# ebarnett2/batotp

Measured on AMD Instinct MI355X. Metric: constraint-evaluated waypoints/sec + traversal-time err vs CPU ref, higher is better.
Workload: dtype f64

## Files before the change

batotp_amd/capi.py:

```python
from __future__ import annotations

import ctypes as C
import os
from typing import Optional, Sequence

import numpy as np

_HERE = os.path.dirname(os.path.abspath(__file__))
_ROOT = os.path.dirname(_HERE)
HIP_LIB_PATH = os.path.join(_HERE, "csrc", "libbatotp_hip.so")

MAX_JOINTS = 8
MAX_CART = 8

ROBOT_KUKA, ROBOT_UR, ROBOT_RR, ROBOT_CSPR3DOF, ROBOT_GENJNT = 1, 2, 3, 4, 5
F_JNT_ACC_ON, F_TRQ_ON, F_CART_VEL_ON, F_CART_ACC_ON = 1 << 0, 1 << 1, 1 << 2, 1 << 3
F_PARALLEL, F_PAR2SER, F_HOST_TRIG, F_NO_SAMPLES, F_COMPACT_SPLINES = 1 << 4, 1 << 5, 1 << 6, 1 << 7, 1 << 8
F_CURVES_IN_PLACE = 1 << 9
F_MVC_IN_CURVES = 1 << 10
F_SVD = 1 << 11
ST_MAX_INTEG_TIME, ST_CAPACITY, ST_BISECT_FAIL = 1 << 0, 1 << 1, 1 << 2
ST_NONFINITE, ST_SHORT, ST_SEG_ERROR = 1 << 3, 1 << 4, 1 << 5

PATH_JOINT, PATH_CART, PATH_BOTH = 1, 2, 3
# ... 767 lines not shown
        self.L.check(self.lib.batotp_hip_output_ms(self.handle, C.byref(v)), "output_ms")
        return float(v.value)


def output_from_rows(ctx: "Context", rows_list, sres, n_theta: int, n_cart: int, n_trq: int) -> Output:
    return Output.from_rows(ctx, rows_list, sres, n_theta, n_cart, n_trq)


def fwdkin_chain(ctx: "Context", chain: KinChain, theta_list: Sequence[np.ndarray], host_trig: bool = True):
    ctx.library.need_kin()
    arrs = [np.ascontiguousarray(t, dtype=np.float64) for t in theta_list]
    for a in arrs:
        assert a.ndim == 2 and a.shape[0] == chain.n_links, (a.shape, chain.n_links)
    n_pts = np.ascontiguousarray([a.shape[1] for a in arrs], dtype=np.int64)
    flat = np.ascontiguousarray(np.concatenate([a.ravel() for a in arrs])) if arrs else np.zeros(0)
    out = np.empty(3 * int(n_pts.sum()), dtype=np.float64)
    ctx.library.check(ctx.library.lib.batotp_hip_fwdkin_chain(ctx.handle, C.byref(chain), F_HOST_TRIG if host_trig else 0, len(arrs),
                                                              n_pts.ctypes.data_as(C.POINTER(C.c_int64)), _dptr(flat), _dptr(out)), "fwdkin_chain")
    res, at = [], 0
    for n in n_pts:
        res.append(out[at: at + 3 * int(n)].reshape(3, int(n)))
        at += 3 * int(n)
    return res


def sdiv_kat(ctx: "Context", a: np.ndarray, b: np.ndarray):
    a = np.ascontiguousarray(a, dtype=np.float64); b = np.ascontiguousarray(b, dtype=np.float64)
    q = np.empty_like(a); w = np.empty(a.size, dtype=np.int32)
    ctx.library.check(ctx.library.lib.batotp_hip_sdiv_kat(ctx.handle, a.size, _dptr(a), _dptr(b), _dptr(q),
                                                          w.ctypes.data_as(C.POINTER(C.c_int32))), "sdiv_kat")
    return q, w.astype(bool)


def out_segmax_kat(ctx: "Context", segs):
    n1 = np.ascontiguousarray([len(x) for x in segs], dtype=np.int32)
    flat = np.ascontiguousarray(np.concatenate([np.asarray(x, dtype=np.int32) for x in segs]), dtype=np.int32)
    ctx.library.check(ctx.library.lib.batotp_hip_out_segmax_kat(ctx.handle, len(segs), n1.ctypes.data_as(C.POINTER(C.c_int32)),
                                                                flat.ctypes.data_as(C.POINTER(C.c_int32))), "out_segmax_kat")
    return np.split(flat, np.cumsum(n1)[:-1])


def spline_lanes_kat(ctx: "Context", y: np.ndarray):
    y = np.ascontiguousarray(y, dtype=np.float64)
    sol, seq = np.empty_like(y), np.empty_like(y)
    redone = C.c_int32(0)
    ctx.library.check(ctx.library.lib.batotp_hip_spline_lanes_kat(ctx.handle, y.size, _dptr(y), _dptr(sol), _dptr(seq), C.byref(redone)),
                      "spline_lanes_kat")
    return sol, seq, int(redone.value)


def div6_kat(ctx: "Context", a: np.ndarray) -> np.ndarray:
    a = np.ascontiguousarray(a, dtype=np.float64)
    q = np.empty_like(a)
    ctx.library.check(ctx.library.lib.batotp_hip_div6_kat(ctx.handle, a.size, _dptr(a), _dptr(q)), "div6_kat")
    return q


class Batch:

    def __init__(self, ctx: Context, prob: Problem, n_knots: Sequence[int], max_steps: int):
        self.ctx, self.lib, self.L = ctx, ctx.library.lib, ctx.library
        self.prob = prob
        self.n_knots = np.ascontiguousarray(n_knots, dtype=np.int64)
        self.n_paths = int(self.n_knots.size)
        self.max_steps = int(max_steps)
        self.handle = C.c_void_p()
# ... 152 lines not shown
```

batotp_amd/csrc/batotp_hip.hip:

```cpp
#include <hip/hip_runtime.h>

#include <algorithm>
#include <cmath>
#include <cstdio>
#include <cstdlib>
#include <cstring>
#include <new>
#include <thread>
#include <type_traits>
#include <vector>

#include "batotp_hip.h"
#include "batotp_models.h"
#include "kernels.hip.h"
#include "sweep1.hip.h"
#include "sweep8.hip.h"
#include "sweep8_fwd.hip.h"
#include "pointwise_va.hip.h"
#include "spline_stream.hip.h"
#include "spline_tile.hip.h"
#include "spline_lanes.hip.h"
#include "resample.hip.h"
#include "output.hip.h"
#include "audit.hip.h"
#include "kin_chain.hip.h"
#include "invdyn.hip.h"
#include "stretch.hip.h"
#include "tscale.hip.h"
#include "stretch_rounds.h"

static inline unsigned seriesBlock(int64_t series)
{
   const int64_t lanes = (series + 255) / 256;
   return (unsigned)(lanes < 4 ? 4 : (lanes > 64 ? 64 : lanes));
}

static inline bool seriesLanesPay(int64_t series) { return series <= 4096; }

using namespace bk;

constexpr int BATOTP_CERT_HOLD_DEFAULT = 3;

static thread_local char g_err[512] = "";

static int hipFail(hipError_t e, const char *what)
// ... 500 lines not shown
   HIP_TRY(hipMemsetAsync(dB, 0xff, sz, st));
   HIP_TRY(hipMemsetAsync(dFlag, 0, sizeof(int), st));
   hipLaunchKernelGGL(k_spline_series_lanes, dim3(1), dim3(64), 0, st, 1, dOff, dOff, dCnt, dy, 1, dA, dFlag);
   HIP_TRY(hipGetLastError());
   hipLaunchKernelGGL(k_spline_series, dim3(1), dim3(seriesBlock(1)), 0, st, 1, dOff, dOff, dCnt, dy, 1, dA, dFlag);
   HIP_TRY(hipGetLastError());
   hipLaunchKernelGGL(k_spline_series, dim3(1), dim3(seriesBlock(1)), 0, st, 1, dOff, dOff, dCnt, dy, 1, dB, (const int *)nullptr);
   HIP_TRY(hipGetLastError());
   HIP_TRY(hipMemcpyAsync(sol, dA, sz, hipMemcpyDeviceToHost, st));
   HIP_TRY(hipMemcpyAsync(sol_seq, dB, sz, hipMemcpyDeviceToHost, st));
   int flag = 0;
   HIP_TRY(hipMemcpyAsync(&flag, dFlag, sizeof(int), hipMemcpyDeviceToHost, st));
   HIP_TRY(hipStreamSynchronize(st));
   *redone = flag;
   return BATOTP_OK;
}

extern "C" int batotp_hip_sdiv_kat(batotp_ctx *ctx, int64_t n, const double *a, const double *b, double *q, int32_t *in_window)
{
   if (!ctx || n <= 0 || !a || !b || !q || !in_window) return BATOTP_ERR_ARG;
   int rc = bind(ctx);
   if (rc) return rc;
   double *d = nullptr;
   const size_t sz = sizeof(double) * (size_t)n;
   HIP_TRY(hipMalloc((void **)&d, 4 * sz));
   hipMemcpyAsync(d, a, sz, hipMemcpyHostToDevice, ctx->stream);
   hipMemcpyAsync(d + n, b, sz, hipMemcpyHostToDevice, ctx->stream);
   hipLaunchKernelGGL(k_kat_sdiv, dim3((unsigned)((n + 255) / 256)), dim3(256), 0, ctx->stream, n, d, d + n, d + 2 * n, reinterpret_cast<int *>(d + 3 * n));
   hipMemcpyAsync(q, d + 2 * n, sz, hipMemcpyDeviceToHost, ctx->stream);
   hipMemcpyAsync(in_window, d + 3 * n, sizeof(int32_t) * (size_t)n, hipMemcpyDeviceToHost, ctx->stream);
   hipError_t e = hipStreamSynchronize(ctx->stream);
   hipFree(d);
   if (e != hipSuccess) return hipFail(e, "sdiv_kat");
   return BATOTP_OK;
}

static int xferReserve(batotp_ctx *ctx, size_t bytes, double **out)
{
   if (ctx->xfer.cap < bytes)
   {
      if (ctx->xfer.p) { hipFree(ctx->xfer.p); ctx->xfer.p = nullptr; ctx->xfer.cap = 0; }
      const size_t want = std::max(bytes, (size_t)1 << 20);
      hipError_t e = hipMalloc(&ctx->xfer.p, want);
      if (e != hipSuccess) { hipFail(e, "hipMalloc(staging)"); (void)hipGetLastError(); return BATOTP_ERR_ALLOC; }
      ctx->xfer.cap = want;
   }
   *out = static_cast<double *>(ctx->xfer.p);
   return BATOTP_OK;
}

static int dynDim(const batotp_problem *prob)
{
   if (!(prob->flags & BATOTP_F_TRQ_ON)) return 0;
   return (prob->flags & BATOTP_F_PARALLEL) ? prob->n_cart : prob->n_joints;
}

extern "C" int batotp_hip_batch_destroy(batotp_batch *b)
{
   if (!b) return BATOTP_OK;
   if (b->ctx) hipSetDevice(b->ctx->device);
   if (b->ctx && b->k3Pending) hipStreamSynchronize(b->ctx->stream2);
   if (b->dFwd == b->dRev) b->dFwd = nullptr;
   void *ptrs[] = {b->dP, b->dPinfo, b->dY, b->dSC, b->dCoef, b->dSamp, b->dDyn, b->dTrig, b->dMvc, b->dRev, b->dFwd, b->dRes, b->dStage, b->dSink, b->dElim, b->dKM, b->dUp, b->dModel, b->dJTrig, b->dTileOff, b->dDirty, b->dEdge, b->dProf, b->dOrder};
   for (void *p : ptrs)
      if (p) hipFree(p);
   for (int k = 0; k < 5; ++k)
// ... 1102 lines not shown
```

batotp_amd/csrc/device_math.h:

```cpp
#pragma once
#include <hip/hip_runtime.h>

namespace bk
{

__device__ __forceinline__ double dmin(double a, double b) { return (b < a) ? b : a; }
__device__ __forceinline__ double dmax(double a, double b) { return (a < b) ? b : a; }
__device__ __forceinline__ int sgn(double v) { return (0.0 < v) - (v < 0.0); }

constexpr double kInf = __builtin_huge_val();

constexpr int DPP_QUAD_XOR1 = 0xB1;
constexpr int DPP_QUAD_XOR2 = 0x4E;
constexpr int DPP_ROW_HALF_MIRROR = 0x141;
constexpr int DPP_ROW_MIRROR = 0x140;
constexpr int DPP_ROW_ROR8 = 0x128;

template <int CTRL>
__device__ __forceinline__ double dpp_mov(double v)
{
   const int lo = __builtin_amdgcn_mov_dpp(__double2loint(v), CTRL, 0xf, 0xf, true);
   const int hi = __builtin_amdgcn_mov_dpp(__double2hiint(v), CTRL, 0xf, 0xf, true);
   return __hiloint2double(hi, lo);
}
template <int CTRL>
__device__ __forceinline__ int dpp_mov(int v)
{
   return __builtin_amdgcn_mov_dpp(v, CTRL, 0xf, 0xf, true);
}

__device__ __forceinline__ double vmin_f64(double a, double b)
{
   double r;
   asm("v_min_f64 %0, %1, %2" : "=v"(r) : "v"(a), "v"(b));
   return r;
}
__device__ __forceinline__ double vmax_f64(double a, double b)
{
   double r;
   asm("v_max_f64 %0, %1, %2" : "=v"(r) : "v"(a), "v"(b));
   return r;
}

template <int G>
__device__ __forceinline__ double grp_min(double v)
{
   if (G == 1) return v;
   v = vmin_f64(v, dpp_mov<DPP_QUAD_XOR1>(v));
   if (G >= 4) v = vmin_f64(v, dpp_mov<DPP_QUAD_XOR2>(v));
   if (G >= 8) v = vmin_f64(v, dpp_mov<DPP_ROW_HALF_MIRROR>(v));
   if (G == 16) v = vmin_f64(v, dpp_mov<DPP_ROW_MIRROR>(v));
   return v;
}
template <int G>
__device__ __forceinline__ double grp_max(double v)
{
   if (G == 1) return v;
   v = vmax_f64(v, dpp_mov<DPP_QUAD_XOR1>(v));
   if (G >= 4) v = vmax_f64(v, dpp_mov<DPP_QUAD_XOR2>(v));
   if (G >= 8) v = vmax_f64(v, dpp_mov<DPP_ROW_HALF_MIRROR>(v));
   if (G == 16) v = vmax_f64(v, dpp_mov<DPP_ROW_MIRROR>(v));
   return v;
}
__device__ __forceinline__ double vmin_f64_raw(double a, double b)
{
   double r;
   asm("v_min_f64 %0, %1, %2" : "=v"(r) : "v"(a), "v"(b));
   return r;
}
__device__ __forceinline__ double vmax_f64_raw(double a, double b)
{
   double r;
   asm("v_max_f64 %0, %1, %2" : "=v"(r) : "v"(a), "v"(b));
   return r;
// ... 64 lines not shown
```

batotp_amd/csrc/sweep8.hip.h:

```cpp
#pragma once
#include "kernels.hip.h"
#include "mvc_window.h"
#include "knot_window.h"

#ifdef S8_PROFILE
#define S8_CNT(k, v) pc[k] += (double)(v)
#define S8_TICK(var) const unsigned long long var = __builtin_readcyclecounter()
#define S8_CYC(k, a, b) pc[k] += (double)((b) - (a))
#else
#define S8_CNT(k, v)
#define S8_TICK(var)
#define S8_CYC(k, a, b)
#endif

namespace bk
{

constexpr int S8_BLOCK = 256;
#define S8_ANY(x) (__builtin_amdgcn_ballot_w64(x) != 0)
#define S8_RARE(x) __builtin_expect(S8_ANY(x), 0)

__device__ __forceinline__ bool s8_ratio_lt_fast(double num, double den, double thr, bool &decided)
{
   const double p = thr * den;
   const bool ok = (p > 1e-290) & (p < 1e290);
   const bool lt = num < p * (1.0 - 1e-14), gt = num > p * (1.0 + 1e-14);
   decided = ok & (lt | gt);
   return lt;
}
__device__ __forceinline__ void s8_ratio_lt_pair(double num1, double num2, double den, bool &lt1, bool &dec1, bool &lt2, bool &dec2)
{
   constexpr double T1 = .001, T2 = 1e-20;
   const bool ok = (den > 1e-260) & (den < 1e260);
   lt1 = num1 < den * (T1 * (1.0 - 1e-14));
   lt2 = num2 < den * (T2 * (1.0 - 1e-14));
   dec1 = ok & (lt1 | (num1 > den * (T1 * (1.0 + 1e-14))));
   dec2 = ok & (lt2 | (num2 > den * (T2 * (1.0 + 1e-14))));
}


__global__ void k_kat_sdiv(int64_t n, const double *__restrict__ a, const double *__restrict__ b, double *__restrict__ q, int *__restrict__ inWindow)
{
   const int64_t i = (int64_t)blockIdx.x * blockDim.x + threadIdx.x;
   if (i >= n) return;
   const bool ok = sdiv_window(a[i]) & sdiv_window(b[i]);
   inWindow[i] = ok ? 1 : 0;
   q[i] = ok ? sdiv_by(a[i], b[i], sdiv_rcp(b[i])) : a[i] / b[i];
}

constexpr int DPP_QUAD_XOR3 = 0x1B;
__device__ __forceinline__ double s8_rcp2(double d)
{
   double r = __builtin_amdgcn_rcp(d);
   r = __builtin_fma(__builtin_fma(-d, r, 1.0), r, r);
   return __builtin_fma(__builtin_fma(-d, r, 1.0), r, r);
}
__device__ __forceinline__ double s8_absmax(double x, double floorv)
{
   double r;
   asm("v_max_f64 %0, |%1|, %2" : "=v"(r) : "v"(x), "v"(floorv));
   return r;
}
__device__ __forceinline__ void s8_certify(bool jOn, double thD, double thD2, double rD, bool rOk, double amaxq, double thrV, double thrA,
                                           double sddotMax, double &lowFact, double &sdotH, double &sdotL, double &sdotTry,
                                           double &sdotGood, int &nGood, int &nIter)
{
   constexpr double BIG = 1e300, TINY = 1e-300;
   const double xTop = sdotH * sdotH;
   const bool use = jOn && !(fabs(thD) < thrV);
   const double aur = amaxq * fabs(rD), mr = thD2 * rD;
   const double er = aur + fabs(mr) * xTop;
   const bool lineOk = rOk & (aur < 1e100) & (fabs(mr) < 1e100) & (er < 1e100);
   const bool have = use & lineOk;
   const double au = have ? aur : BIG;
   const double mj = have ? mr : 0.0;
   const double ej = use ? (lineOk ? er : kInf) : 0.0;
   const double uMin = grp_min<8>(au);
   const double eMax = grp_max<8>(ej);
   const double sMin2 = dmin(uMin, sddotMax);
   const bool standing = jOn && !use && !(fabs(thD2) < thrA);
   double xForce = kInf;
   if (S8_RARE(standing)) xForce = grp_min<8>(standing ? amaxq / fabs(thD2) : kInf);
   double xs = (au + sddotMax) * s8_rcp2(s8_absmax(mj, TINY));
#define S8_PAIR(AUI, MI) xs = vmin_f64(xs, (au + (AUI)) * s8_rcp2(s8_absmax(mj - (MI), TINY)))
   {
      const double a1 = dpp_mov<DPP_QUAD_XOR1>(au), m1 = dpp_mov<DPP_QUAD_XOR1>(mj);
      S8_PAIR(a1, m1);
      const double a2 = dpp_mov<DPP_QUAD_XOR2>(au), m2 = dpp_mov<DPP_QUAD_XOR2>(mj);
      S8_PAIR(a2, m2);
      const double a3 = dpp_mov<DPP_QUAD_XOR3>(au), m3 = dpp_mov<DPP_QUAD_XOR3>(mj);
      S8_PAIR(a3, m3);
      const double a7 = dpp_mov<DPP_ROW_HALF_MIRROR>(au), m7 = dpp_mov<DPP_ROW_HALF_MIRROR>(mj);
      S8_PAIR(a7, m7);
      const double a6 = dpp_mov<DPP_QUAD_XOR1>(a7), m6 = dpp_mov<DPP_QUAD_XOR1>(m7);
      S8_PAIR(a6, m6);
      const double a5 = dpp_mov<DPP_QUAD_XOR2>(a7), m5 = dpp_mov<DPP_QUAD_XOR2>(m7);
      S8_PAIR(a5, m5);
      const double a4 = dpp_mov<DPP_QUAD_XOR3>(a7), m4 = dpp_mov<DPP_QUAD_XOR3>(m7);
      S8_PAIR(a4, m4);
   }
#undef S8_PAIR
   xs = grp_min<8>(xs);
   const double xstar = dmin(xs, 4.0 * xTop);
   const double R = eMax * s8_rcp2(sMin2 > 0.0 ? sMin2 : 1.0);
   const double band = (R * 0x1p-40) * xstar;
   const bool forceFirst = xForce < xstar - band;
   const double xThr = forceFirst ? xForce : xstar;
   const double bandThr = forceFirst ? -1.0 : band;
   const bool sane = (sddotMax == sddotMax) & (eMax == eMax) & (xstar == xstar) & (R == R) & (R < 0x1p30) & (sMin2 > 1e-100) & (eMax < 1e100) &
                     (xTop > 1e-100) & (xTop < 1e100) & (xstar > 1e-100) & (forceFirst | (xForce > xstar + band));
   if (sane)
   {
      int it = nIter;
      bool inBand = false, more = true;
      for (;;)
      {
         const double c = sdotTry, d = c * c - xThr;
         inBand = !((fabs(d) > bandThr) & (c > 1e-100));
         more = more & !inBand & (d > 0.0) & (it < 90);
         if (!S8_ANY(more)) break;
         const double lf2 = lowFact * 2.0;
         const double lo = dmax(.999 * 0.0, (1.0 - lf2) * c);
         lowFact = more ? lf2 : lowFact;
         sdotH = more ? c : sdotH;
         sdotL = more ? lo : sdotL;
         sdotTry = .5 * (sdotH + sdotL);
         it += more ? 1 : 0;
      }
      const bool bisect = !inBand & (it < 90);
      sdotGood = bisect ? sdotTry : sdotGood;
      nGood = bisect ? 1 : nGood;
      sdotL = bisect ? sdotTry : sdotL;
      it += bisect ? 1 : 0;
      sdotTry = .5 * (sdotH + sdotL);
      const double convThr = 1e-3 * (1.0 + 3e-14);
      more = bisect;
      for (;;)
      {
         const double c = sdotTry, d = c * c - xThr;
         const bool viol = d > 0.0;
         const bool goesOn = viol | (fabs(c - sdotL) > convThr * c);
         more = more & (fabs(d) > bandThr) & goesOn & (it < 90);
         if (!S8_ANY(more)) break;
         sdotH = (more & viol) ? c : sdotH;
         sdotL = (more & !viol) ? c : sdotL;
         sdotTry = .5 * (sdotH + sdotL);
         it += more ? 1 : 0;
      }
      sdotGood = bisect ? sdotL : sdotGood;
      nIter = it;
   }
}

template <int G, int FEAT, int DIR>
__global__ void __launch_bounds__(S8_BLOCK, G == 8 ? 2 : 1) k_sweep8(SweepArgs a)
{
   static_assert(FEAT == -1 || FEAT == 0, "velocity / acceleration-only problems");
   static_assert(G == 8 || G == 4, "lanes per path");
   constexpr int PER = 8 / G;
   __shared__ double lim[6][8];
   __shared__ double rk[7][6];
   __shared__ double2 pts[S8_BLOCK / G][4];
   __shared__ double2 vw[S8_BLOCK / G][8];
   if (threadIdx.x < 42)
   {
      const double tab[42] = {0, 0, 0, 0, 0, 0,
                              BK_B00, 0, 0, 0, 0, 0,
                              BK_B01, BK_B11, 0, 0, 0, 0,
                              BK_B02, BK_B12, BK_B22, 0, 0, 0,
                              BK_B03, BK_B13, BK_B23, BK_B33, 0, 0,
                              BK_B04, BK_B14, BK_B24, BK_B34, BK_B44, 0,
                              BK_B05, BK_B15, BK_B25, BK_B35, BK_B45, BK_B55};
      (&rk[0][0])[threadIdx.x] = tab[threadIdx.x];
   }
   stage_limits(a.dP, lim);

// ... 103 lines not shown
   unsigned status = t.status;
   int nfail = t.nfail;
   double sdotCur = t.sdotCur;
   double sddotL = t.sddotL, sddotH = t.sddotH;

   double v1 = 0, v2 = 0, v3 = 0, v4 = 0, v5 = 0;
   double w1 = 0, w2 = 0, w3 = 0, w4 = 0, w5 = 0, w6 = 0;
   double sPrev = s0v, sdPrev = v0, sCurPt = s0v, sdCurPt = v0;
   double sCur = s0v;

   const int iMax = (maxIntegSteps > 0x3ffffff0) ? 0x3ffffff0 : (int)maxIntegSteps;
   const int capI = (int)cap;
   const int revStartI = (revStart > 0x3fffffff) ? 0x3fffffff : (int)revStart;
#define S8_CURVE_FULL(i) ((i) >= capI || (DIR == 1 && (i) + 64 >= revStartI + segM))

   {
      const int idx0 = (DIR == 1) ? 0 : capI - 1;
      if (writer) { out[idx0] = make_double2(s0v, v0); mypts[idx0 & 3] = make_double2(s0v, v0); }
   }
   int flushedTo = (DIR == 1) ? 0 : capI;

   const double floorV = 0.0 / absh;
   int nPts = 0, i = 1;
   unsigned endStatus = 0;
   int st = (DIR == 1) ? -1 : 0;
   constexpr int PH_FIRST = 0, PH_ENDED = 1, PH_CHECK = 2, PH_DEAD = 3, PH_CERT = 4;
   constexpr bool CERT = DIR == -1 && PER == 1;
   const int holdC = a.holdc;
   int phase = PH_ENDED;
   if (S8_CURVE_FULL(i)) { endStatus = BATOTP_ST_CAPACITY; phase = PH_DEAD; }
   double sN = 0, wN = 0;
   double lowFact = .01, sdotGood = 0, sdotL = 0, sdotH = 0, sdotTry = 0;
   int nGood = 0, nIter = 0;
   bool wild = !(fabs(v0) < kInf) | !(fabs(w0) < kInf);
   bool stageFailed = false;
   const int hold = a.hold;
#ifdef S8_PROFILE
   double pc[16];
   for (int k = 0; k < 16; ++k) pc[k] = 0;
   const unsigned long long tLoop0 = __builtin_readcyclecounter();
#endif

   for (;;)
   {
      const unsigned long long mAlive = __ballot(phase != PH_DEAD);
      if (mAlive == 0) break;
      const unsigned long long mWait = __ballot(phase < PH_CHECK);
      const bool startNow = (mWait == mAlive) || (__popcll(mWait) * 8 >= __popcll(mAlive) * hold);
      S8_CNT(0, 1); S8_CNT(13, __popcll(mAlive) / G);
      if (CERT)
      {
         const unsigned long long mCert = __ballot(phase == PH_CERT);
         if (mCert != 0)
         {
            const bool progress = (startNow && mWait != 0) || ((mAlive & ~mWait & ~mCert) != 0);
            if (__popcll(mCert) * 8 >= __popcll(mAlive) * holdC || !progress)
            {
               S8_TICK(tF0);
               S8_CNT(11, 1); S8_CNT(15, __popcll(mCert) / G);
               if (phase == PH_CERT)
               {
                  s8_certify(jOn[0], thD[0], thD2[0], rD[0], rOk[0], amax[0], thrV, thrA, sddotMax, lowFact, sdotH, sdotL, sdotTry, sdotGood,
                             nGood, nIter);
                  phase = PH_CHECK;
               }
               S8_TICK(tF1);
               S8_CYC(14, tF0, tF1);
            }
         }
      }
      S8_TICK(tA);
      if (startNow && mWait != 0)
      {
         S8_CNT(1, 1); S8_CNT(2, __popcll(mWait) / G);
         if (phase < PH_CHECK)
         {
            {
               phase = PH_FIRST;
               const double vN = sdotCur;
               wild |= !(fabs(vN) < kInf) | !(fabs(wN) < kInf);
               {
                  double *slotV = reinterpret_cast<double *>(myvw + ((unsigned)st < 6u ? st : 7));
                  double *slotW = reinterpret_cast<double *>(myvw + (((unsigned)st < 6u && !stageFailed) ? st : 7)) + 1;
                  *slotV = vN;
                  *slotW = wN;
               }
               const bool stepEnd = (st == 6);
               st = stepEnd ? st : st + 1;
               if (S8_ANY(stepEnd))
               {
                  S8_CNT(8, 1);
                  if (stepEnd)
                  {
                     const double wE = stageFailed ? w6 : wN;
                     s0v = sN; v0 = vN; w0 = wE; w6 = wE;
                     sPrev = sCurPt; sdPrev = sdCurPt;
                     sCurPt = s0v; sdCurPt = v0;
                     const int idx = (DIR == 1) ? i : capI - 1 - i;
                     mypts[idx & 3] = make_double2(s0v, v0);
                     st = (DIR == 1) ? 0 : 1;
                     const bool fin = sCur * DIR > sLast;
                     const bool late = !fin && (i > iMax);
                     nPts = fin ? i + 1 : nPts;
                     i = (fin || late) ? i : i + 1;
                     const bool full = !fin && !late && S8_CURVE_FULL(i);
                     endStatus = late ? (unsigned)BATOTP_ST_MAX_INTEG_TIME : (full ? (unsigned)BATOTP_ST_CAPACITY : endStatus);
                     phase = (fin || late || full) ? PH_DEAD : phase;
                     const bool chunk = !fin && ((DIR == 1) ? ((idx & 3) == 3) : ((idx & 3) == 0));
                     if (S8_ANY(chunk))
                     {
                        if (chunk)
                        {
                           const int base = idx & ~3;
// ... 20 lines not shown
                        st = 1;
                     }
                  }
               }
               const double *bc = rk[st];
               double sdotT = 0, sddotT = 0;
               {
                  const double2 q1 = myvw[1], q2 = myvw[2], q3 = myvw[3], q4 = myvw[4], q5 = myvw[5];
                  v1 = q1.x; w1 = q1.y; v2 = q2.x; w2 = q2.y; v3 = q3.x; w3 = q3.y; v4 = q4.x; w4 = q4.y; v5 = q5.x; w5 = q5.y;
               }
               bool slowDiv = false;
#pragma unroll
               for (int q = 0; q < PER; ++q) slowDiv |= jOn[q] && fabs(thD[q]) > thrV && !(rOk[q] & sdiv_window(vmax[q]));
               const bool odd = S8_RARE(wild | slowDiv);
               if (!odd)
               {
                  sdotT += bc[0] * v0; sddotT += bc[0] * w0;
                  sdotT += bc[1] * v1; sddotT += bc[1] * w1;
                  sdotT += bc[2] * v2; sddotT += bc[2] * w2;
                  sdotT += bc[3] * v3; sddotT += bc[3] * w3;
                  sdotT += bc[4] * v4; sddotT += bc[4] * w4;
                  sdotT += bc[5] * v5; sddotT += bc[5] * w5;
               }
               else
               {
                  sdotT += bc[0] * v0; sddotT += bc[0] * w0;
                  { const double a1 = sdotT + bc[1] * v1, b1 = sddotT + bc[1] * w1; sdotT = (st > 1) ? a1 : sdotT; sddotT = (st > 1) ? b1 : sddotT; }
                  { const double a2 = sdotT + bc[2] * v2, b2 = sddotT + bc[2] * w2; sdotT = (st > 2) ? a2 : sdotT; sddotT = (st > 2) ? b2 : sddotT; }
                  { const double a3 = sdotT + bc[3] * v3, b3 = sddotT + bc[3] * w3; sdotT = (st > 3) ? a3 : sdotT; sddotT = (st > 3) ? b3 : sddotT; }
                  { const double a4 = sdotT + bc[4] * v4, b4 = sddotT + bc[4] * w4; sdotT = (st > 4) ? a4 : sdotT; sddotT = (st > 4) ? b4 : sddotT; }
                  { const double a5 = sdotT + bc[5] * v5, b5 = sddotT + bc[5] * w5; sdotT = (st > 5) ? a5 : sdotT; sddotT = (st > 5) ? b5 : sddotT; }
               }
               sN = s0v + h * sdotT;
               double vN = v0 + h * sddotT;
               vN = dmax(vN, floorV);
               sCur = sN;

               if (DIR == 1)
               {
#include "sweep8_mvcwalk.inc"
                  const double tauM = (sCur - mS0) / (mS1 - mS0);
                  const double sdotMVC = dmax(mD0 + tauM * (mD1 - mD0), sdotMin);
                  vN = (vN > sdotMVC) ? sdotMVC : vN;
               }
               vN = dmin(vN, sdotCap);
               vN = dmax(vN, sdotMin);
               double lim1 = kInf;
               {
#pragma unroll
                  for (int q = 0; q < PER; ++q)
                  {
                     const bool on = jOn[q] && fabs(thD[q]) > thrV;
                     const bool fast = rOk[q] & sdiv_window(vmax[q]);
                     const double qv = fabs(sdiv_by(vmax[q], thD[q], rD[q]));
                     lim1 = (on & fast) ? dmin(lim1, qv) : lim1;
                  }
                  if (odd)
                  {
#pragma unroll
                     for (int q = 0; q < PER; ++q)
                     {
                        const bool on = jOn[q] && fabs(thD[q]) > thrV;
                        const bool fast = rOk[q] & sdiv_window(vmax[q]);
                        if (on && !fast) lim1 = dmin(lim1, fabs(vmax[q] / thD[q]));
                     }
                  }
                  lim1 = grp_min<G>(lim1);
                  vN = dmin(vN, lim1);
               }
               sdotCur = vN;
               lowFact = .01; sdotGood = 0; nGood = 0; sdotL = 0; sdotH = vN; sdotTry = vN; nIter = 0; stageFailed = false;

               if (S8_ANY(!((sCur >= sSeg) & (sCur <= sNext))))
               {
                  S8_CNT(10, 1);
                  for (;;)
                  {
                     sSeg = sres * (double)seg;
                     sNext = sres * (double)(seg + 1);
                     const bool inside = (sCur >= sSeg) & (sCur <= sNext);
                     const bool up = !inside & (sCur > sSeg), down = !inside & (sCur < sSeg);
                     status |= (!inside & !up & !down) ? (unsigned)BATOTP_ST_NONFINITE : 0u;
                     const bool mvUp = up & (seg < lastSeg), mvDn = down & (seg > 0);
                     seg = mvUp ? seg + 1 : (mvDn ? seg - 1 : seg);
                     if (!S8_ANY(mvUp | mvDn)) break;
                  }
               }
               double tau = (sCur - sSeg) / (sNext - sSeg);
               const bool chg = (seg != rowSeg);
               if (S8_ANY(chg))
               {
                  S8_CNT(9, 1);
                  if (chg)
                  {
#pragma unroll
                     for (int q = 0; q < PER; ++q)
                     {
                        if (FEAT < 0)
                        {
                           const unsigned at = (unsigned)(seg * nIn + jAt[q]);
                           double yL = (DIR == 1) ? kEdgeY[q] : kPreY[q], solL = (DIR == 1) ? kEdgeSol[q] : kPreSol[q];
// ... 254 lines not shown
```

batotp_amd/csrc/sweep8_fwd.hip.h:

```cpp
#pragma once
#include "sweep8.hip.h"
#include <type_traits>

namespace bk
{

template <int FEAT>
__global__ void __launch_bounds__(S8_BLOCK, 2) k_sweep8_lock(SweepArgs a)
{
   static_assert(FEAT == -1 || FEAT == 0, "velocity / acceleration-only problems");
   constexpr int G = 8, DIR = 1;
   __shared__ double lim[6][8];
   __shared__ double2 pts[S8_BLOCK / G][4];
   const double rkB[6][6] = {{BK_B00, 0, 0, 0, 0, 0},
                             {BK_B01, BK_B11, 0, 0, 0, 0},
                             {BK_B02, BK_B12, BK_B22, 0, 0, 0},
                             {BK_B03, BK_B13, BK_B23, BK_B33, 0, 0},
                             {BK_B04, BK_B14, BK_B24, BK_B34, BK_B44, 0},
                             {BK_B05, BK_B15, BK_B25, BK_B35, BK_B45, BK_B55}};
   stage_limits(a.dP, lim);

   const int lane = threadIdx.x & 63;
   const int wave = blockIdx.x * (S8_BLOCK / 64) + (threadIdx.x >> 6);
   const int j = lane % G;
// ... 23 lines not shown
   t.mvc = reinterpret_cast<const double *>(mvc);
   t.nMvc = nMvc;
   const int64_t revStart = (a.fwd == a.rev) ? cap - (int64_t)nMvc : ((int64_t)1 << 62);

   const double absh = pi.integ_res;
   const double h = absh;
   const int64_t maxIntegSteps = (int64_t)floor(a.P.max_integ_time / pi.integ_res) + 1;
   const double sres = pi.sres_c;
   const double sEnd = sres * (double)(n - 1);
   double s0v = 0.0;
   double v0, w0 = 0;
   t.segC = 0; t.tauC = 0; t.segMVC = 0; t.tauMVC = 0;
   t.sCur = s0v;
   t.sdotCur = 0;
#pragma unroll 1
   for (int pass = 0; pass < 2; ++pass)
   {
      accel_pt(t, j, w0);
      if (pass == 0) { v0 = .1 * h * w0; t.sdotMin = v0; }
      else v0 = t.sdotCur;
      sdot_lim(t, j, v0);
      if (pass == 0) { t.sdotMin = v0; t.sdotCur = v0; }
   }
   const double vBoot = v0;

   const bool jOn = j < t.nJ;
   const int jAt = jOn ? j : 0;
   const double vmax = t.vmax[0], amax = t.amax[0];
   double c1 = jOn ? t.rowTh[0].c1 : 0.0, c2x2 = jOn ? 2 * t.rowTh[0].c2 : 0.0;
   double c3x3 = jOn ? 3 * t.rowTh[0].c3 : 0.0, c3x6 = jOn ? 6 * t.rowTh[0].c3 : 0.0;
   double thD = t.thD[0], thD2 = t.thD2[0];
   bool rOk = sdiv_window(thD);
   double rD = sdiv_rcp(thD);
   const bool accOn = (t.flags & BATOTP_F_JNT_ACC_ON) != 0;
   const double thrV = t.thrV, thrA = t.thrA, vfact = t.vfact, afact = t.afact;
   const double sdotCap = t.sdotCap, sddotMax = t.sddotMax, sdotMin = t.sdotMin;
   const bool capOk = (sddotMax == sddotMax);
   const int lastSeg = n - 2;
   const int nIn = t.nIn;
   const double2 *__restrict__ km = t.km;
   const double *__restrict__ coef = t.coef;
   const int rowStride = t.C * 4;
   int seg = t.segC, rowSeg = t.rowSeg;
   double kEdgeY = 0, kEdgeSol = 0, kPreY = 0, kPreSol = 0;
   int preIdx = KNOT_WINDOW_NONE;
   int segM = t.segMVC;
   double mS0, mD0, mS1, mD1, mSLo, mDLo, mSHi, mDHi;
   {
      const double2 qa = mvc[segM], qb = mvc[segM + 1], ql = mvc[mvc_window_lo(segM)], qh = mvc[mvc_window_hi(segM, nMvc)];
      mS0 = qa.x; mD0 = qa.y; mS1 = qb.x; mD1 = qb.y;
      mSLo = ql.x; mDLo = ql.y; mSHi = qh.x; mDHi = qh.y;
   }
   unsigned status = t.status;
   int nfail = t.nfail;
   double sdotCur = t.sdotCur;
   double sddotH = t.sddotH;

   double v1 = 0, v2 = 0, v3 = 0, v4 = 0, v5 = 0;
   double w1 = 0, w2 = 0, w3 = 0, w4 = 0, w5 = 0, w6 = 0;
   double sCur = s0v;

   const int iMax = (maxIntegSteps > 0x3ffffff0) ? 0x3ffffff0 : (int)maxIntegSteps;
   const int capI = (int)cap;
   const int revStartI = (revStart > 0x3fffffff) ? 0x3fffffff : (int)revStart;
#define S8L_CURVE_FULL(i) ((i) >= capI || (i) + 64 >= revStartI + segM)

   if (writer) { out[0] = make_double2(s0v, v0); mypts[0] = make_double2(s0v, v0); }

   const double floorV = 0.0 / absh;
   int i = 1;
   unsigned endStatus = 0;
   bool alive = true;
   if (S8L_CURVE_FULL(i)) { endStatus = BATOTP_ST_CAPACITY; alive = false; }
   double sN = 0, wN = 0;
   double lowFact = .01, sdotGood = 0, sdotL = 0, sdotH = 0, sdotTry = 0;
   int nGood = 0, nIter = 0;
   bool stageFailed = false;
#ifdef S8_PROFILE
   double pc[16];
   for (int k = 0; k < 16; ++k) pc[k] = 0;
   const unsigned long long tLoop0 = __builtin_readcyclecounter();
#endif

   auto checkPass = [&](auto firstTag, bool &more) -> bool {
      constexpr bool FIRST = decltype(firstTag)::value;
      const double lowFact2 = lowFact * 2.0;
      const double sdotLShrunk = dmax(.999 * 0.0, (1.0 - lowFact2) * sdotTry);
      bool dec1, dec2;
      const double num1 = fabs(sdotTry - sdotGood), num2 = sdotTry - sdotLShrunk;
      bool close, tiny;
      s8_ratio_lt_pair(num1, num2, sdotTry, close, dec1, tiny, dec2);
      const double sdotSQ = sdotTry * sdotTry;
      double H = sddotMax, L = -sddotMax;
      bool force = false;
      if (accOn)
      {
         const bool slow = fabs(thD) < thrV;
         const double vTerm = thD2 * sdotSQ;
         const double sa = (thD < 0.0) ? -amax : amax;
         const double nH = sa - vTerm, nL = -sa - vTerm;
         const bool fast = capOk & rOk & sdiv_window(nH) & sdiv_window(nL);
         const double qH = sdiv_by(nH, thD, rD);
// ... 55 lines not shown
               S8_CNT(11, 1);
               if (ffWant)
                  s8_certify(jOn, thD, thD2, rD, rOk, amax, thrV, thrA, sddotMax, lowFact, sdotH, sdotL, sdotTry, sdotGood, nGood, nIter);
            }
         }
         if (FIRST) more = S8_ANY(!(fin || failed));
      }
      wN = fin ? sddotH : wN;
      return fin || failed;
   };

   for (;;)
   {
      if (!S8_ANY(alive)) break;
      if (alive)
      {
         sCur = s0v + h * v0;
#include "sweep8_mvcwalk.inc"
#pragma unroll
         for (int st = 1; st <= 6; ++st)
         {
            S8_TICK(tA);
            S8_CNT(1, 1); S8_CNT(2, __popcll(__ballot(1)) / G);
            const double *bc = rkB[st - 1];
            const double b0 = bc[0], b1 = bc[1], b2 = bc[2], b3 = bc[3], b4 = bc[4], b5 = bc[5];
            double sdotT = 0, sddotT = 0;
            sdotT += b0 * v0; sddotT += b0 * w0;
            if (st > 1) { sdotT += b1 * v1; sddotT += b1 * w1; }
            if (st > 2) { sdotT += b2 * v2; sddotT += b2 * w2; }
            if (st > 3) { sdotT += b3 * v3; sddotT += b3 * w3; }
            if (st > 4) { sdotT += b4 * v4; sddotT += b4 * w4; }
            if (st > 5) { sdotT += b5 * v5; sddotT += b5 * w5; }
            sN = s0v + h * sdotT;
            double vN = v0 + h * sddotT;
            vN = dmax(vN, floorV);
            sCur = sN;

            {
#include "sweep8_mvcwalk.inc"
               const double tauM = (sCur - mS0) / (mS1 - mS0);
               const double sdotMVC = dmax(mD0 + tauM * (mD1 - mD0), sdotMin);
               vN = (vN > sdotMVC) ? sdotMVC : vN;
            }
            vN = dmin(vN, sdotCap);
            vN = dmax(vN, sdotMin);
            {
               double lim1 = kInf;
               const bool on = jOn && fabs(thD) > thrV;
               const bool fast = rOk & sdiv_window(vmax);
               const double qv = fabs(sdiv_by(vmax, thD, rD));
               lim1 = (on & fast) ? dmin(lim1, qv) : lim1;
               if (S8_RARE(on & !fast))
               {
                  if (on && !fast) lim1 = dmin(lim1, fabs(vmax / thD));
               }
               lim1 = grp_min<G>(lim1);
               vN = dmin(vN, lim1);
            }
            sdotCur = vN;
            lowFact = .01; sdotGood = 0; nGood = 0; sdotL = 0; sdotH = vN; sdotTry = vN; nIter = 0; stageFailed = false;

            double sSeg = sres * (double)seg, sNext = sres * (double)(seg + 1);
            if (S8_ANY(!((sCur >= sSeg) & (sCur <= sNext))))
            {
               S8_CNT(10, 1);
               for (;;)
               {
                  sSeg = sres * (double)seg;
                  sNext = sres * (double)(seg + 1);
                  const bool inside = (sCur >= sSeg) & (sCur <= sNext);
                  const bool up = !inside & (sCur > sSeg), down = !inside & (sCur < sSeg);
                  status |= (!inside & !up & !down) ? (unsigned)BATOTP_ST_NONFINITE : 0u;
                  const bool mvUp = up & (seg < lastSeg), mvDn = down & (seg > 0);
                  seg = mvUp ? seg + 1 : (mvDn ? seg - 1 : seg);
                  if (!S8_ANY(mvUp | mvDn)) break;
               }
            }
            const double tau = (sCur - sSeg) / (sNext - sSeg);
            const bool chg = (seg != rowSeg);
            if (S8_ANY(chg))
            {
               S8_CNT(9, 1);
               if (chg)
               {
                  if (FEAT < 0)
                  {
                     const unsigned at = (unsigned)(seg * nIn + jAt);
                     double yL = kEdgeY, solL = kEdgeSol, yR = kPreY, solR = kPreSol;
                     bool literal = !knot_window_hit(preIdx, seg, DIR);
                     const double xa = solR - solL, xb = solR + 2 * solL;
// ... 7 lines not shown
                     if (S8_RARE(literal))
                     {
                        const bool hit = knot_window_hit(preIdx, seg, DIR);
                        const double2 dl = km[at], dr = km[at + nIn];
                        yL = hit ? yL : dl.x; solL = hit ? solL : dl.y;
                        yR = hit ? yR : dr.x; solR = hit ? solR : dr.y;
                        c3 = div6(solR - solL);
                        sixthB = div6(solR + 2 * solL);
                     }
                     knot_window_shift(true, DIR, yL, solL, yR, solR, kEdgeY, kEdgeSol);
                     const double c2 = solL / 2.0;
                     c1 = yR - yL - sixthB;
                     c2x2 = 2 * c2; c3x3 = 3 * c3; c3x6 = 6 * c3;
                     preIdx = knot_window_mark(seg, lastSeg, DIR);
                  }
                  else
                  {
                     const Coef4 k = *reinterpret_cast<const Coef4 *>(coef + (unsigned)(seg * rowStride) + jAt * 4);
                     c1 = k.c1; c2x2 = 2 * k.c2; c3x3 = 3 * k.c3; c3x6 = 6 * k.c3;
                  }
                  rowSeg = seg;
               }
               if (FEAT < 0)
               {
                  const double2 kq = km[(unsigned)(knot_window_load(seg, lastSeg, DIR) * nIn + jAt)];
                  kPreY = kq.x; kPreSol = kq.y;
               }
            }
            {
               const double tau2 = tau * tau;
               thD = (c3x3 * tau2 + c2x2 * tau + c1) * vfact;
               thD2 = (c3x6 * tau + c2x2) * afact;
               rOk = sdiv_window(thD);
               rD = sdiv_rcp(thD);
            }
            S8_TICK(tB);
            S8_CYC(5, tA, tB);

            S8_CNT(0, 1); S8_CNT(3, 1); S8_CNT(4, __popcll(__ballot(1)) / G); S8_CNT(13, __popcll(__ballot(1)) / G);
            bool more;
            bool ended = checkPass(std::true_type(), more);
            while (more)
            {
               S8_CNT(0, 1); S8_CNT(3, 1); S8_CNT(4, __popcll(__ballot(!ended)) / G); S8_CNT(13, __popcll(__ballot(1)) / G);
               if (!ended)
               {
                  bool unused;
                  ended = checkPass(std::false_type(), unused);
               }
               more = S8_ANY(!ended);
            }
            S8_TICK(tC);
            S8_CYC(6, tB, tC);

            if (st == 1) { v1 = sdotCur; w1 = stageFailed ? w1 : wN; }
            if (st == 2) { v2 = sdotCur; w2 = stageFailed ? w2 : wN; }
            if (st == 3) { v3 = sdotCur; w3 = stageFailed ? w3 : wN; }
            if (st == 4) { v4 = sdotCur; w4 = stageFailed ? w4 : wN; }
            if (st == 5) { v5 = sdotCur; w5 = stageFailed ? w5 : wN; }
         }
         {
            S8_CNT(8, 1);
            const double vN = sdotCur;
            const double wE = stageFailed ? w6 : wN;
            s0v = sN; v0 = vN; w0 = wE; w6 = wE;
            const int idx = i;
// ... 82 lines not shown
```

batotp_amd/csrc/sweep8_mvcwalk.inc:

```
{
   for (;;)
   {
      const MvcMove mvM = mvc_window_test(sCur, segM, nMvc, mS0, mS1);
      status |= mvM.status;
      if (!S8_ANY(mvM.up | mvM.dn)) break;
      mvc_window_shift(mvM, segM, mSLo, mDLo, mS0, mD0, mS1, mD1, mSHi, mDHi);
      const double2 qLoM = mvc[mvc_window_lo(segM)], qHiM = mvc[mvc_window_hi(segM, nMvc)];
      mSLo = qLoM.x; mDLo = qLoM.y; mSHi = qHiM.x; mDHi = qHiM.y;
   }
}
```

Before: 362.4 million.

## Use raw v_min/v_max clamp chain with ballot-guarded literal fallback

Replaces the velocity clamp chain in the forward and backward sweeps with raw v_min_f64/v_max_f64 instructions. The slow literal path (exact NaN semantics, non-window division) runs only when a combined wave ballot flags a rare lane, and loop-exit tests now build per-condition ballot masks instead of carrying a 'more' flag. The wild-value check is widened to cover very large finite values, h, and the clamp constants, so the fast path can assume ordinary inputs. A known-answer test kernel and a Python binding are added to compare the literal and fast clamps. This trades more ballot instructions per step for fewer compare/select sequences, and relies on the NaN-handling differences being caught by the masks.

Result: faster. 369.6 million, median of 6 (+2.0%).

```diff
diff --git a/batotp_amd/capi.py b/batotp_amd/capi.py
--- a/batotp_amd/capi.py
+++ b/batotp_amd/capi.py
@@ -823,6 +823,20 @@
     return q, w.astype(bool)
 
 
+def clamp_kat(ctx: "Context", raw, interp, cap, smin, lim1):
+    arrs = [np.ascontiguousarray(a, dtype=np.float64) for a in (raw, interp, cap, smin, lim1)]
+    n = arrs[0].size
+    assert all(a.size == n for a in arrs)
+    fn = ctx.library.lib.batotp_hip_clamp_kat
+    D = C.POINTER(C.c_double)
+    fn.argtypes = [C.c_void_p, C.c_int64, D, D, D, D, D, D, D, C.POINTER(C.c_int32)]
+    fn.restype = C.c_int
+    literal = np.empty(n); fast = np.empty(n); valid = np.empty(n, dtype=np.int32)
+    ctx.library.check(fn(ctx.handle, n, *[_dptr(a) for a in arrs], _dptr(literal), _dptr(fast),
+                         valid.ctypes.data_as(C.POINTER(C.c_int32))), "clamp_kat")
+    return literal, fast, valid.astype(bool)
+
+
 def out_segmax_kat(ctx: "Context", segs):
     n1 = np.ascontiguousarray([len(x) for x in segs], dtype=np.int32)
     flat = np.ascontiguousarray(np.concatenate([np.asarray(x, dtype=np.int32) for x in segs]), dtype=np.int32)
diff --git a/batotp_amd/csrc/batotp_hip.hip b/batotp_amd/csrc/batotp_hip.hip
--- a/batotp_amd/csrc/batotp_hip.hip
+++ b/batotp_amd/csrc/batotp_hip.hip
@@ -11,6 +11,7 @@
 #include <vector>
 
 #include "batotp_hip.h"
+#include "batotp_hip_clamp_kat.h"
 #include "batotp_models.h"
 #include "kernels.hip.h"
 #include "sweep1.hip.h"
@@ -577,6 +578,28 @@
    hipError_t e = hipStreamSynchronize(ctx->stream);
    hipFree(d);
    if (e != hipSuccess) return hipFail(e, "sdiv_kat");
+   return BATOTP_OK;
+}
+
+extern "C" int batotp_hip_clamp_kat(batotp_ctx *ctx, int64_t n, const double *raw, const double *interp, const double *cap, const double *smin,
+                                    const double *lim1, double *literal, double *fast, int32_t *valid)
+{
+   if (!ctx || n <= 0 || !raw || !interp || !cap || !smin || !lim1 || !literal || !fast || !valid) return BATOTP_ERR_ARG;
+   int rc = bind(ctx);
+   if (rc) return rc;
+   double *d = nullptr;
+   const size_t sz = sizeof(double) * (size_t)n;
+   HIP_TRY(hipMalloc((void **)&d, 8 * sz));
+   struct Guard { double *p; ~Guard() { if (p) (void)hipFree(p); } } guard{d};
+   const double *in[5] = {raw, interp, cap, smin, lim1};
+   for (int k = 0; k < 5; ++k) HIP_TRY(hipMemcpyAsync(d + k * n, in[k], sz, hipMemcpyHostToDevice, ctx->stream));
+   hipLaunchKernelGGL(k_kat_clamp, dim3((unsigned)((n + 255) / 256)), dim3(256), 0, ctx->stream, n, d, d + n, d + 2 * n, d + 3 * n, d + 4 * n,
+                      d + 5 * n, d + 6 * n, reinterpret_cast<int *>(d + 7 * n));
+   HIP_TRY(hipGetLastError());
+   HIP_TRY(hipMemcpyAsync(literal, d + 5 * n, sz, hipMemcpyDeviceToHost, ctx->stream));
+   HIP_TRY(hipMemcpyAsync(fast, d + 6 * n, sz, hipMemcpyDeviceToHost, ctx->stream));
+   HIP_TRY(hipMemcpyAsync(valid, d + 7 * n, sizeof(int32_t) * (size_t)n, hipMemcpyDeviceToHost, ctx->stream));
+   HIP_TRY(hipStreamSynchronize(ctx->stream));
    return BATOTP_OK;
 }
 
diff --git a/batotp_amd/csrc/device_math.h b/batotp_amd/csrc/device_math.h
--- a/batotp_amd/csrc/device_math.h
+++ b/batotp_amd/csrc/device_math.h
@@ -40,6 +40,32 @@
    double r;
    asm("v_max_f64 %0, %1, %2" : "=v"(r) : "v"(a), "v"(b));
    return r;
+}
+
+__device__ __forceinline__ bool clamp_consts_ok(double floorV, double sdotMin, double sdotCap)
+{
+   return (floorV == floorV) & (sdotMin > 0.0) & (sdotCap == sdotCap);
+}
+__device__ __forceinline__ bool clamp_raw_ok(double raw, double interp) { return !__builtin_isunordered(raw, interp); }
+template <bool FWD>
+__device__ __forceinline__ double clamp_chain_literal(double raw, double interp, double floorV, double sdotMin, double sdotCap)
+{
+   double vN = dmax(raw, floorV);
+   if (FWD)
+   {
+      const double sdotMVC = dmax(interp, sdotMin);
+      vN = (vN > sdotMVC) ? sdotMVC : vN;
+   }
+   vN = dmin(vN, sdotCap);
+   return dmax(vN, sdotMin);
+}
+template <bool FWD>
+__device__ __forceinline__ double clamp_chain_fast(double raw, double interp, double floorV, double sdotMin, double sdotCap)
+{
+   double vN = vmax_f64(raw, floorV);
+   if (FWD) vN = vmin_f64(vN, vmax_f64(interp, sdotMin));
+   vN = vmin_f64(vN, sdotCap);
+   return vmax_f64(vN, sdotMin);
 }
 
 template <int G>
diff --git a/batotp_amd/csrc/sweep8.hip.h b/batotp_amd/csrc/sweep8.hip.h
--- a/batotp_amd/csrc/sweep8.hip.h
+++ b/batotp_amd/csrc/sweep8.hip.h
@@ -19,6 +19,10 @@
 constexpr int S8_BLOCK = 256;
 #define S8_ANY(x) (__builtin_amdgcn_ballot_w64(x) != 0)
 #define S8_RARE(x) __builtin_expect(S8_ANY(x), 0)
+typedef unsigned long long s8_mask;
+#define S8_MASK(cmp) __builtin_amdgcn_ballot_w64(cmp)
+#define S8_EXEC() __builtin_amdgcn_ballot_w64(true)
+#define S8_MASK_WINDOW(x) (S8_MASK(fabs(x) >= SDIV_LO) & S8_MASK(fabs(x) <= SDIV_HI))
 
 __device__ __forceinline__ bool s8_ratio_lt_fast(double num, double den, double thr, bool &decided)
 {
@@ -38,7 +42,6 @@
    dec2 = ok & (lt2 | (num2 > den * (T2 * (1.0 + 1e-14))));
 }
 
-
 __global__ void k_kat_sdiv(int64_t n, const double *__restrict__ a, const double *__restrict__ b, double *__restrict__ q, int *__restrict__ inWindow)
 {
    const int64_t i = (int64_t)blockIdx.x * blockDim.x + threadIdx.x;
@@ -46,6 +49,18 @@
    const bool ok = sdiv_window(a[i]) & sdiv_window(b[i]);
    inWindow[i] = ok ? 1 : 0;
    q[i] = ok ? sdiv_by(a[i], b[i], sdiv_rcp(b[i])) : a[i] / b[i];
+}
+
+__global__ void k_kat_clamp(int64_t n, const double *__restrict__ raw, const double *__restrict__ interp, const double *__restrict__ cap,
+                            const double *__restrict__ smin, const double *__restrict__ lim1, double *__restrict__ literal,
+                            double *__restrict__ fast, int *__restrict__ valid)
+{
+   const int64_t i = (int64_t)blockIdx.x * blockDim.x + threadIdx.x;
+   if (i >= n) return;
+   const double floorV = 0.0;
+   valid[i] = (clamp_consts_ok(floorV, smin[i], cap[i]) & clamp_raw_ok(raw[i], interp[i])) ? 1 : 0;
+   literal[i] = dmin(clamp_chain_literal<true>(raw[i], interp[i], floorV, smin[i], cap[i]), lim1[i]);
+   fast[i] = vmin_f64(clamp_chain_fast<true>(raw[i], interp[i], floorV, smin[i], cap[i]), lim1[i]);
 }
 
 constexpr int DPP_QUAD_XOR3 = 0x1B;
@@ -112,13 +127,14 @@
    if (sane)
    {
       int it = nIter;
-      bool inBand = false, more = true;
+      bool inBand = false;
       for (;;)
       {
          const double c = sdotTry, d = c * c - xThr;
          inBand = !((fabs(d) > bandThr) & (c > 1e-100));
-         more = more & !inBand & (d > 0.0) & (it < 90);
-         if (!S8_ANY(more)) break;
+         const bool more = (fabs(d) > bandThr) & (c > 1e-100) & (d > 0.0) & (it < 90);
+         const s8_mask mMore = S8_MASK(fabs(d) > bandThr) & S8_MASK(c > 1e-100) & S8_MASK(d > 0.0) & S8_MASK(it < 90);
+         if (mMore == 0) break;
          const double lf2 = lowFact * 2.0;
          const double lo = dmax(.999 * 0.0, (1.0 - lf2) * c);
          lowFact = more ? lf2 : lowFact;
@@ -128,20 +144,22 @@
          it += more ? 1 : 0;
       }
       const bool bisect = !inBand & (it < 90);
+      const s8_mask mBisect = S8_MASK(fabs(sdotTry * sdotTry - xThr) > bandThr) & S8_MASK(sdotTry > 1e-100) & S8_MASK(it < 90);
       sdotGood = bisect ? sdotTry : sdotGood;
       nGood = bisect ? 1 : nGood;
       sdotL = bisect ? sdotTry : sdotL;
       it += bisect ? 1 : 0;
       sdotTry = .5 * (sdotH + sdotL);
       const double convThr = 1e-3 * (1.0 + 3e-14);
-      more = bisect;
       for (;;)
       {
          const double c = sdotTry, d = c * c - xThr;
          const bool viol = d > 0.0;
-         const bool goesOn = viol | (fabs(c - sdotL) > convThr * c);
-         more = more & (fabs(d) > bandThr) & goesOn & (it < 90);
-         if (!S8_ANY(more)) break;
+         const double gap = fabs(c - sdotL), thr = convThr * c;
+         const bool goesOn = viol | (gap > thr);
+         const bool more = bisect & (fabs(d) > bandThr) & goesOn & (it < 90);
+         const s8_mask mMore = mBisect & S8_MASK(fabs(d) > bandThr) & (S8_MASK(d > 0.0) | S8_MASK(gap > thr)) & S8_MASK(it < 90);
+         if (mMore == 0) break;
          sdotH = (more & viol) ? c : sdotH;
          sdotL = (more & !viol) ? c : sdotL;
          sdotTry = .5 * (sdotH + sdotL);
@@ -311,7 +329,8 @@
    double sN = 0, wN = 0;
    double lowFact = .01, sdotGood = 0, sdotL = 0, sdotH = 0, sdotTry = 0;
    int nGood = 0, nIter = 0;
-   bool wild = !(fabs(v0) < kInf) | !(fabs(w0) < kInf);
+   constexpr double S8_ORDINARY = 1e290;
+   bool wild = !(fabs(v0) < S8_ORDINARY) | !(fabs(w0) < S8_ORDINARY) | !(fabs(h) < kInf) | !clamp_consts_ok(floorV, sdotMin, sdotCap);
    bool stageFailed = false;
    const int hold = a.hold;
 #ifdef S8_PROFILE
@@ -357,7 +376,7 @@
             {
                phase = PH_FIRST;
                const double vN = sdotCur;
-               wild |= !(fabs(vN) < kInf) | !(fabs(wN) < kInf);
+               wild |= !(fabs(vN) < S8_ORDINARY) | !(fabs(wN) < S8_ORDINARY);
                {
                   double *slotV = reinterpret_cast<double *>(myvw + ((unsigned)st < 6u ? st : 7));
                   double *slotW = reinterpret_cast<double *>(myvw + (((unsigned)st < 6u && !stageFailed) ? st : 7)) + 1;
@@ -444,19 +463,21 @@
                   { const double a5 = sdotT + bc[5] * v5, b5 = sddotT + bc[5] * w5; sdotT = (st > 5) ? a5 : sdotT; sddotT = (st > 5) ? b5 : sddotT; }
                }
                sN = s0v + h * sdotT;
-               double vN = v0 + h * sddotT;
-               vN = dmax(vN, floorV);
+               const double vRaw = v0 + h * sddotT;
                sCur = sN;
 
+               double vN = vmax_f64(vRaw, floorV);
+               double sdotRev = 0;
                if (DIR == 1)
                {
 #include "sweep8_mvcwalk.inc"
                   const double tauM = (sCur - mS0) / (mS1 - mS0);
-                  const double sdotMVC = dmax(mD0 + tauM * (mD1 - mD0), sdotMin);
+                  sdotRev = mD0 + tauM * (mD1 - mD0);
+                  const double sdotMVC = dmax(sdotRev, sdotMin);
                   vN = (vN > sdotMVC) ? sdotMVC : vN;
                }
-               vN = dmin(vN, sdotCap);
-               vN = dmax(vN, sdotMin);
+               vN = vmin_f64(vN, sdotCap);
+               vN = vmax_f64(vN, sdotMin);
                double lim1 = kInf;
                {
 #pragma unroll
@@ -469,6 +490,7 @@
                   }
                   if (odd)
                   {
+                     vN = clamp_chain_literal<DIR == 1>(vRaw, sdotRev, floorV, sdotMin, sdotCap);
 #pragma unroll
                      for (int q = 0; q < PER; ++q)
                      {
@@ -476,9 +498,14 @@
                         const bool fast = rOk[q] & sdiv_window(vmax[q]);
                         if (on && !fast) lim1 = dmin(lim1, fabs(vmax[q] / thD[q]));
                      }
-                  }
-                  lim1 = grp_min<G>(lim1);
-                  vN = dmin(vN, lim1);
+                     lim1 = grp_min<G>(lim1);
+                     vN = dmin(vN, lim1);
+                  }
+                  else
+                  {
+                     lim1 = grp_min<G>(lim1);
+                     vN = vmin_f64(vN, lim1);
+                  }
                }
                sdotCur = vN;
                lowFact = .01; sdotGood = 0; nGood = 0; sdotL = 0; sdotH = vN; sdotTry = vN; nIter = 0; stageFailed = false;
diff --git a/batotp_amd/csrc/sweep8_fwd.hip.h b/batotp_amd/csrc/sweep8_fwd.hip.h
--- a/batotp_amd/csrc/sweep8_fwd.hip.h
+++ b/batotp_amd/csrc/sweep8_fwd.hip.h
@@ -79,6 +79,8 @@
    double thD = t.thD[0], thD2 = t.thD2[0];
    bool rOk = sdiv_window(thD);
    double rD = sdiv_rcp(thD);
+   s8_mask mROk = S8_MASK_WINDOW(thD);
+   const s8_mask mJOn = S8_MASK(j < t.nJ), mVmaxOk = S8_MASK_WINDOW(vmax);
    const bool accOn = (t.flags & BATOTP_F_JNT_ACC_ON) != 0;
    const double thrV = t.thrV, thrA = t.thrA, vfact = t.vfact, afact = t.afact;
    const double sdotCap = t.sdotCap, sddotMax = t.sddotMax, sdotMin = t.sdotMin;
@@ -115,6 +117,7 @@
    if (writer) { out[0] = make_double2(s0v, v0); mypts[0] = make_double2(s0v, v0); }
 
    const double floorV = 0.0 / absh;
+   const s8_mask mClampLit = ~(S8_MASK(floorV == floorV) & S8_MASK(sdotMin > 0.0) & S8_MASK(sdotCap == sdotCap));
    int i = 1;
    unsigned endStatus = 0;
    bool alive = true;
@@ -236,30 +239,26 @@
             if (st > 4) { sdotT += b4 * v4; sddotT += b4 * w4; }
             if (st > 5) { sdotT += b5 * v5; sddotT += b5 * w5; }
             sN = s0v + h * sdotT;
-            double vN = v0 + h * sddotT;
-            vN = dmax(vN, floorV);
+            const double vRaw = v0 + h * sddotT;
             sCur = sN;
 
-            {
 #include "sweep8_mvcwalk.inc"
-               const double tauM = (sCur - mS0) / (mS1 - mS0);
-               const double sdotMVC = dmax(mD0 + tauM * (mD1 - mD0), sdotMin);
-               vN = (vN > sdotMVC) ? sdotMVC : vN;
-            }
-            vN = dmin(vN, sdotCap);
-            vN = dmax(vN, sdotMin);
+            const double tauM = (sCur - mS0) / (mS1 - mS0);
+            const double sdotRev = mD0 + tauM * (mD1 - mD0);
+            double vN = clamp_chain_fast<true>(vRaw, sdotRev, floorV, sdotMin, sdotCap);
             {
                double lim1 = kInf;
                const bool on = jOn && fabs(thD) > thrV;
                const bool fast = rOk & sdiv_window(vmax);
                const double qv = fabs(sdiv_by(vmax, thD, rD));
                lim1 = (on & fast) ? dmin(lim1, qv) : lim1;
-               if (S8_RARE(on & !fast))
+               vN = vmin_f64(vN, grp_min<G>(lim1));
+               const s8_mask mRareV = (mJOn & S8_MASK(fabs(thD) > thrV) & ~(mROk & mVmaxOk)) | (mClampLit & S8_EXEC()) | S8_MASK(!clamp_raw_ok(vRaw, sdotRev));
+               if (__builtin_expect(mRareV != 0, 0))
                {
                   if (on && !fast) lim1 = dmin(lim1, fabs(vmax / thD));
+                  vN = dmin(clamp_chain_literal<true>(vRaw, sdotRev, floorV, sdotMin, sdotCap), grp_min<G>(lim1));
                }
-               lim1 = grp_min<G>(lim1);
-               vN = dmin(vN, lim1);
             }
             sdotCur = vN;
             lowFact = .01; sdotGood = 0; nGood = 0; sdotL = 0; sdotH = vN; sdotTry = vN; nIter = 0; stageFailed = false;
@@ -333,6 +332,7 @@
                thD = (c3x3 * tau2 + c2x2 * tau + c1) * vfact;
                thD2 = (c3x6 * tau + c2x2) * afact;
                rOk = sdiv_window(thD);
+               mROk = S8_MASK_WINDOW(thD);
                rD = sdiv_rcp(thD);
             }
             S8_TICK(tB);
diff --git a/batotp_amd/csrc/sweep8_mvcwalk.inc b/batotp_amd/csrc/sweep8_mvcwalk.inc
--- a/batotp_amd/csrc/sweep8_mvcwalk.inc
+++ b/batotp_amd/csrc/sweep8_mvcwalk.inc
@@ -3,7 +3,9 @@
    {
       const MvcMove mvM = mvc_window_test(sCur, segM, nMvc, mS0, mS1);
       status |= mvM.status;
-      if (!S8_ANY(mvM.up | mvM.dn)) break;
+      const s8_mask mUpM = S8_MASK(sCur > mS0) & S8_MASK(!(sCur <= mS1)) & S8_MASK(segM < nMvc - 2);
+      const s8_mask mDnM = S8_MASK(sCur < mS0) & S8_MASK(segM > 0);
+      if ((mUpM | mDnM) == 0) break;
       mvc_window_shift(mvM, segM, mSLo, mDLo, mS0, mD0, mS1, mD1, mSHi, mDHi);
       const double2 qLoM = mvc[mvc_window_lo(segM)], qHiM = mvc[mvc_window_hi(segM, nMvc)];
       mSLo = qLoM.x; mDLo = qLoM.y; mSHi = qHiM.x; mDHi = qHiM.y;
diff --git a/include/batotp_hip_clamp_kat.h b/include/batotp_hip_clamp_kat.h
--- /dev/null
+++ b/include/batotp_hip_clamp_kat.h
@@ -0,0 +1,17 @@
+#ifndef BATOTP_HIP_CLAMP_KAT_H
+#define BATOTP_HIP_CLAMP_KAT_H
+
+#include "batotp_hip.h"
+
+#ifdef __cplusplus
+extern "C" {
+#endif
+
+int batotp_hip_clamp_kat(batotp_ctx *ctx, int64_t n, const double *raw, const double *interp, const double *cap, const double *smin,
+                         const double *lim1, double *literal, double *fast, int32_t *valid);
+
+#ifdef __cplusplus
+}
+#endif
+
+#endif
```
